# study-game-engines/directx-renderer-kurth

Hardware: AMD Instinct MI355X
Metric: physics steps/sec at 100k rigid bodies (higher is better)
Workload: dtype f32; 1 GPU; c3: 100k mixed colliders (sphere/capsule/OBB), dt 1/120 s, 30 solver iterations; bodies=100000, broadphase_pairs=611032, manifolds=251275, contacts=317267, joints=0, recoveries=0, parallelism=1 gpu

## Files before the change

directx-renderer-kurth_amd/csrc/k_broad.hip:

```cpp
#include "world.h"
#include <rocprim/rocprim.hpp>

#define CELL_BIAS (1 << 20)
#define CELL_MASK ((1u << 21) - 1u)
#define EMPTY_CELL 0xFFFFFFFFu

MI_DEV u64 packCell(i32 ix, i32 iy, i32 iz) { return ((u64)(u32)(ix & CELL_MASK)) | ((u64)(u32)(iy & CELL_MASK) << 21) | ((u64)(u32)(iz & CELL_MASK) << 42); }
MI_DEV u32 hashCell(u64 k, u32 mask)
{
	k ^= k >> 30; k *= 0xbf58476d1ce4e5b9ull; k ^= k >> 27; k *= 0x94d049bb133111ebull; k ^= k >> 31;
	return (u32)k & mask;
}
MI_DEV i32 cellCoord(float v, float invCell)
{
	float c = floorf(v * invCell);
	c = fminf(fmaxf(c, -(float)(CELL_BIAS - 2)), (float)(CELL_BIAS - 2));
	return (i32)c + CELL_BIAS;
}
MI_DEV u32 cellTag(i32 ix, i32 iy, i32 iz) { return ((u32)ix & 0x3FFu) | (((u32)iy & 0x3FFu) << 10) | (((u32)iz & 0x3FFu) << 20); }
MI_DEV bool aabbOverlap(float4 amin, float4 amax, float4 bmin, float4 bmax)
{
	if (amax.x < bmin.x || amin.x > bmax.x) return false;
	if (amax.y < bmin.y || amin.y > bmax.y) return false;
	if (amax.z < bmin.z || amin.z > bmax.z) return false;
	return true;
}

__global__ void __launch_bounds__(256) k_cell_assign(const u32* __restrict__ activeCols, u32 hashMask, const float4* __restrict__ aabbMin, const float4* __restrict__ aabbMax,
	u32* __restrict__ counters, u32* __restrict__ hashKey, u32* __restrict__ cellCount)
{
	const u32 gid = blockIdx.x * blockDim.x + threadIdx.x;
	if (gid == 0) { counters[CTR_FIRST_LARGE] = 0xFFFFFFFFu; counters[CTR_FIRST_INACTIVE] = 0xFFFFFFFFu; counters[CTR_PAIR_OVERFLOW] = 0u; }
	const u32 n = counters[CTR_ACTIVE_COLS];
	float maxExtent = fmaxf(__uint_as_float(counters[CTR_CELL_SIZE]), 1e-3f);
	float cell = maxExtent * 1.001f;
	float invCell = 1.f / cell;
	for (u32 a = gid; a < n; a += gridDim.x * blockDim.x)
	{
		const u32 i = activeCols[a];
		float4 mn = aabbMin[i], mx = aabbMax[i];
		float e = fmaxf(fmaxf(mx.x - mn.x, mx.y - mn.y), mx.z - mn.z);
		u32 h;
		if (mn.x > mx.x) { h = hashMask + 2; }
		else if (e > maxExtent) { h = hashMask + 1; }
		else { h = hashCell(packCell(cellCoord(mn.x, invCell), cellCoord(mn.y, invCell), cellCoord(mn.z, invCell)), hashMask); }
		hashKey[i] = h;
		atomicAdd(&cellCount[h], 1u);
	}
}

__global__ void __launch_bounds__(256) k_cell_place(const u32* __restrict__ counters, const u32* __restrict__ activeCols, const u32* __restrict__ hashKey, u32* __restrict__ cellBase, u32* __restrict__ tmpIdx)
{
	const u32 n = counters[CTR_ACTIVE_COLS];
	for (u32 a = blockIdx.x * blockDim.x + threadIdx.x; a < n; a += gridDim.x * blockDim.x) { const u32 i = activeCols[a]; tmpIdx[atomicAdd(&cellBase[hashKey[i]], 1u)] = i; }
}
__global__ void __launch_bounds__(256) k_cell_rank(u32* __restrict__ counters, u32 hashMask, const u32* __restrict__ hashKey, const u32* __restrict__ cellBase, const u32* __restrict__ cellCount, const u32* __restrict__ tmpIdx,
	const float4* __restrict__ aabbMin, const float4* __restrict__ aabbMax, float4* __restrict__ sBox, u32* __restrict__ cellRange)
{
	const u32 n = counters[CTR_ACTIVE_COLS];
	const float cell = fmaxf(__uint_as_float(counters[CTR_CELL_SIZE]), 1e-3f) * 1.001f;
	const float invCell = 1.f / cell;
	if (blockIdx.x == 0 && threadIdx.x == 0) counters[CTR_CELL_SIZE_USED] = counters[CTR_CELL_SIZE];
	for (u32 t = blockIdx.x * blockDim.x + threadIdx.x; t < n; t += gridDim.x * blockDim.x)
	{
		const u32 i = tmpIdx[t], h = hashKey[i], end = cellBase[h], start = end - cellCount[h];
		u32 rank = t - start;
		if (h != hashMask + 2u) { rank = 0; for (u32 u = start; u < end; ++u) rank += tmpIdx[u] < i ? 1u : 0u; }
		const u32 pos = start + rank;
		float4 mn = aabbMin[i], mx = aabbMax[i];
		mx.w = __uint_as_float(cellTag(cellCoord(mn.x, invCell), cellCoord(mn.y, invCell), cellCoord(mn.z, invCell)));
		mn.w = __uint_as_float(i);
		sBox[2 * pos] = mn; sBox[2 * pos + 1] = mx;
		if (t == start)
		{
			if (h <= hashMask) { cellRange[2 * h] = start; cellRange[2 * h + 1] = end; }
			else counters[h == hashMask + 1 ? CTR_FIRST_LARGE : CTR_FIRST_INACTIVE] = start;
		}
	}
}

#define PAIR_SLAB 32
#define PAIR_LANES 16
enum { MODE_SLAB = 0, MODE_WRITE = 1 };
template <int MODE>
__global__ void __launch_bounds__(256) k_pairs(u32 nc, u32 hashMask, const float4* __restrict__ sBox, const uint2* __restrict__ cellRange, u32* __restrict__ counters,
	u32* __restrict__ pairCount, const u32* __restrict__ pairOffset, uint2* __restrict__ out, u32 pairCap)
{
	u32 gid = blockIdx.x * blockDim.x + threadIdx.x;
	u32 t = gid / PAIR_LANES, g = gid % PAIR_LANES;
	bool valid = t < nc;
	u32 nEnd = min(counters[CTR_FIRST_INACTIVE], min(nc, counters[CTR_ACTIVE_COLS]));
	u32 firstLarge = min(counters[CTR_FIRST_LARGE], nEnd);
	bool live = valid && t < nEnd;
	if (MODE == MODE_WRITE) live = live && pairCount[t] > PAIR_SLAB;
	float4 amin = make_float4(0.f, 0.f, 0.f, 0.f), amax = amin;
	u32 me = 0;
	u32 s = 0, e = 0; u32 ntag = 0; bool checkKey = false;
	if (live)
	{
		amin = sBox[2 * t]; amax = sBox[2 * t + 1];
		me = __float_as_uint(amin.w);
		if (t >= firstLarge) { if (g == 0) { s = firstLarge; e = t; } }
		else if (g == 14) { s = firstLarge; e = nEnd; }
		else if (g < 14)
		{
			const float invCell = 1.f / (fmaxf(__uint_as_float(counters[CTR_CELL_SIZE_USED]), 1e-3f) * 1.001f);
			i32 ix = cellCoord(amin.x, invCell), iy = cellCoord(amin.y, invCell), iz = cellCoord(amin.z, invCell);
			i32 o = 13 + (i32)g;
			i32 dz = o / 9 - 1, dy = (o / 3) % 3 - 1, dx = o % 3 - 1;
			ntag = cellTag(ix + dx, iy + dy, iz + dz);
			u32 h = hashCell(packCell(ix + dx, iy + dy, iz + dz), hashMask);
			uint2 range = cellRange[h];
			if (range.x != EMPTY_CELL)
			{
				s = range.x; e = range.y;
				if (g == 0) e = min(e, t);
				checkKey = true;
			}
		}
	}
	u32 n = 0;
	u32 hit0 = 0, hit1 = 0, hit2 = 0, hit3 = 0;
	for (u32 u = s; u < e; u += 4u)
	{
		float4 bmin[4], bmax[4];
#pragma unroll
		for (u32 k = 0; k < 4u; ++k) if (u + k < e) { bmin[k] = sBox[2 * (u + k)]; bmax[k] = sBox[2 * (u + k) + 1]; }
#pragma unroll
		for (u32 k = 0; k < 4u; ++k)
		{
			if (u + k >= e) continue;
			if (checkKey && __float_as_uint(bmax[k].w) != ntag) continue;
			if (aabbOverlap(amin, amax, bmin[k], bmax[k]))
			{
				u32 partner = __float_as_uint(bmin[k].w);
				if (n == 0) hit0 = partner; else if (n == 1) hit1 = partner; else if (n == 2) hit2 = partner; else if (n == 3) hit3 = partner;
				++n;
			}
		}
	}
	u32 incl = n;
	for (u32 d = 1; d < PAIR_LANES; d <<= 1) { u32 v = __shfl_up(incl, d, PAIR_LANES); if (g >= d) incl += v; }
	u32 total = __shfl(incl, PAIR_LANES - 1, PAIR_LANES);
	u32 pos = incl - n;
	if (MODE == MODE_SLAB && valid && g == 0) { pairCount[t] = live ? total : 0; if (total > PAIR_SLAB) counters[CTR_PAIR_OVERFLOW] = 1; }
	if (!n) return;
	size_t base = (MODE == MODE_WRITE) ? (size_t)pairOffset[t] : (size_t)t * PAIR_SLAB;
	u32 room = (MODE == MODE_WRITE) ? 0xFFFFFFFFu : PAIR_SLAB;
	if (n <= 4)
	{
		for (u32 k = 0; k < n; ++k)
		{
			u32 partner = k == 0 ? hit0 : (k == 1 ? hit1 : (k == 2 ? hit2 : hit3));
			if (pos + k < room && (MODE == MODE_SLAB || base + pos + k < pairCap)) out[base + pos + k] = make_uint2(me, partner);
		}
		return;
	}
	for (u32 u = s; u < e; ++u)
	{
		float4 bmin = sBox[2 * u], bmax = sBox[2 * u + 1];
		if (checkKey && __float_as_uint(bmax.w) != ntag) continue;
		if (!aabbOverlap(amin, amax, bmin, bmax)) continue;
		if (pos < room && (MODE == MODE_SLAB || base + pos < pairCap)) out[base + pos] = make_uint2(me, __float_as_uint(bmin.w));
		++pos;
	}
}

__global__ void __launch_bounds__(256) k_pairs_pack(u32 nc, const u32* __restrict__ pairCount, const u32* __restrict__ pairOffset, const uint2* __restrict__ slab,
	uint2* __restrict__ pairs, u32 pairCap)
{
	u32 i = blockIdx.x * blockDim.x + threadIdx.x;
	u32 t = i / PAIR_SLAB, k = i % PAIR_SLAB;
	if (t >= nc || k >= pairCount[t]) return;
	u32 dst = pairOffset[t] + k;
	if (dst < pairCap) pairs[dst] = slab[i];
}

__global__ void k_finish_pair_count(u32 launched, const u32* __restrict__ pairCount, const u32* __restrict__ pairOffset, u32* __restrict__ counters, const double* __restrict__ sapPartial, u32 sapBlocks, u32 stepParity)
{
	double acc[7] = { 0., 0., 0., 0., 0., 0., 0. };
	for (u32 b = threadIdx.x; b < sapBlocks; b += 64u) for (int k = 0; k < 7; ++k) acc[k] += sapPartial[(size_t)b * 7 + k];
	for (int o = 32; o > 0; o >>= 1) for (int k = 0; k < 7; ++k) acc[k] += __shfl_xor(acc[k], o);
	if (threadIdx.x == 0 && blockIdx.x == 0)
	{
		const u32 na = counters[CTR_ACTIVE_COLS], nc = min(na, launched);
		counters[CTR_ACTIVE_OVERFLOW] = na > launched ? 1u : 0u;
		counters[CTR_NUM_PAIRS] = nc ? pairOffset[nc - 1] + pairCount[nc - 1] : 0;
		counters[CTR_CELL_SIZE] = 0;
		const double n = acc[6] > 0. ? acc[6] : 1.;
		const double vx = acc[3] - acc[0] * acc[0] / n, vy = acc[4] - acc[1] * acc[1] / n, vz = acc[5] - acc[2] * acc[2] / n;
		counters[CTR_SAP_AXIS + (stepParity ^ 1u)] = (vx > vy) ? ((vx > vz) ? 0u : 2u) : ((vy > vz) ? 1u : 2u);
	}
}

static void ensureTemp(World& w, size_t bytes)
{
	if (bytes > w.tempStorage.cap) w.tempStorage.ensure(bytes + bytes / 2 + 4096, w.stream);
}
void prim_sort_pairs_u32(World& w, const u32* kin, u32* kout, const u32* vin, u32* vout, u32 n, u32 bits)
{
	if (!n) return;
	size_t bytes = 0;
	MI_CHECK(rocprim::radix_sort_pairs(nullptr, bytes, kin, kout, vin, vout, n, 0, bits, w.stream));
	ensureTemp(w, bytes);
	MI_CHECK(rocprim::radix_sort_pairs(w.tempStorage.p, bytes, kin, kout, vin, vout, n, 0, bits, w.stream));
}
void prim_sort_pairs_u32_u64(World& w, const u32* kin, u32* kout, const u64* vin, u64* vout, u32 n, u32 bits)
{
	if (!n) return;
	size_t bytes = 0;
	MI_CHECK(rocprim::radix_sort_pairs(nullptr, bytes, kin, kout, vin, vout, n, 0, bits, w.stream));
	ensureTemp(w, bytes);
	MI_CHECK(rocprim::radix_sort_pairs(w.tempStorage.p, bytes, kin, kout, vin, vout, n, 0, bits, w.stream));
}
void prim_exclusive_scan_u32(World& w, const u32* in, u32* out, u32 n)
{
	if (!n) return;
	size_t bytes = 0;
	MI_CHECK(rocprim::exclusive_scan(nullptr, bytes, in, out, 0u, n, rocprim::plus<u32>(), w.stream));
	ensureTemp(w, bytes);
	MI_CHECK(rocprim::exclusive_scan(w.tempStorage.p, bytes, in, out, 0u, n, rocprim::plus<u32>(), w.stream));
}

static u32 log2ceil(u32 v) { u32 b = 0; while ((1u << b) < v) ++b; return b; }

void launch_broadphase_count(World& w)
{
	if (!w.nc) return;
	const u32 bound = (u32)std::min<u64>(w.nc, (u64)w.estActiveCols + w.estActiveCols / 8u + 2048u);
	w.pairBound = bound;
	dim3 grid(std::max(1u, (bound + 255u) / 256u)), block(256);
	u32 H = w.hashTableSize, mask = H - 1;
	hipLaunchKernelGGL(k_cell_assign, grid, block, 0, w.stream, w.actCols.p, mask, w.aabbMin.p, w.aabbMax.p, w.dCounters.p, w.hashKey.p, w.cellCount.p);
	prim_exclusive_scan_u32(w, w.cellCount.p, w.cellBase.p, H + 3);
	hipLaunchKernelGGL(k_cell_place, grid, block, 0, w.stream, w.dCounters.p, w.actCols.p, w.hashKey.p, w.cellBase.p, w.sortIdx.p);
	hipLaunchKernelGGL(k_cell_rank, grid, block, 0, w.stream, w.dCounters.p, mask, w.hashKey.p, w.cellBase.p, w.cellCount.p, w.sortIdx.p, w.aabbMin.p, w.aabbMax.p, w.sBox.p, w.cellStart.p);
	w.pairSlab.ensure((size_t)bound * PAIR_SLAB, w.stream);
	if (w.lastError) return;
	hipLaunchKernelGGL(HIP_KERNEL_NAME(k_pairs<MODE_SLAB>), dim3((u32)(((size_t)bound * PAIR_LANES + 255) / 256)), block, 0, w.stream, bound, mask, w.sBox.p, (const uint2*)w.cellStart.p, w.dCounters.p,
		w.pairCount.p, w.pairOffset.p, w.pairSlab.p, 0u);
	prim_exclusive_scan_u32(w, w.pairCount.p, w.pairOffset.p, bound);
	hipLaunchKernelGGL(k_finish_pair_count, dim3(1), dim3(64), 0, w.stream, bound, w.pairCount.p, w.pairOffset.p, w.dCounters.p, w.sapPartial.p, w.sapBlocks, w.stats.numInternalSteps & 1u);
}

void launch_broadphase_write(World& w, u32 numPairs, bool slabOverflow)
{
	const u32 nc = w.pairBound;
	if (!nc || !numPairs) return;
	hipLaunchKernelGGL(k_pairs_pack, dim3((u32)(((size_t)nc * PAIR_SLAB + 255) / 256)), dim3(256), 0, w.stream, nc, w.pairCount.p, w.pairOffset.p, w.pairSlab.p, w.pairs.p, (u32)w.pairCap);
	if (slabOverflow)
		hipLaunchKernelGGL(HIP_KERNEL_NAME(k_pairs<MODE_WRITE>), dim3((u32)(((size_t)nc * PAIR_LANES + 255) / 256)), dim3(256), 0, w.stream, nc, w.hashTableSize - 1, w.sBox.p, (const uint2*)w.cellStart.p, w.dCounters.p, w.pairCount.p, w.pairOffset.p, w.pairs.p, (u32)w.pairCap);
}
```

Before: 528.2 steps/s.

## Balance broadphase pair scan across lanes and skip unreachable neighbor cells

```diff
diff --git a/directx-renderer-kurth_amd/csrc/k_broad.hip b/directx-renderer-kurth_amd/csrc/k_broad.hip
--- a/directx-renderer-kurth_amd/csrc/k_broad.hip
+++ b/directx-renderer-kurth_amd/csrc/k_broad.hip
@@ -81,13 +81,18 @@
 
 #define PAIR_SLAB 32
 #define PAIR_LANES 16
+#define PAIR_NO_TAG 0xFFFFFFFFu
 enum { MODE_SLAB = 0, MODE_WRITE = 1 };
+MI_DEV uint2 pairRange(const uint4* ranges, u32 r) { return make_uint2(ranges[r].x, ranges[r].y); }
+MI_DEV const float4* pairBox(const float4* __restrict__ sBox, u32 u) { return (const float4*)((const char*)sBox + u * 32u); }
 template <int MODE>
 __global__ void __launch_bounds__(256) k_pairs(u32 nc, u32 hashMask, const float4* __restrict__ sBox, const uint2* __restrict__ cellRange, u32* __restrict__ counters,
 	u32* __restrict__ pairCount, const u32* __restrict__ pairOffset, uint2* __restrict__ out, u32 pairCap)
 {
+	__shared__ uint4 sRange[256 / PAIR_LANES][PAIR_LANES];
 	u32 gid = blockIdx.x * blockDim.x + threadIdx.x;
 	u32 t = gid / PAIR_LANES, g = gid % PAIR_LANES;
+	const uint4* __restrict__ ranges = sRange[threadIdx.x / PAIR_LANES];
 	bool valid = t < nc;
 	u32 nEnd = min(counters[CTR_FIRST_INACTIVE], min(nc, counters[CTR_ACTIVE_COLS]));
 	u32 firstLarge = min(counters[CTR_FIRST_LARGE], nEnd);
@@ -95,47 +100,69 @@
 	if (MODE == MODE_WRITE) live = live && pairCount[t] > PAIR_SLAB;
 	float4 amin = make_float4(0.f, 0.f, 0.f, 0.f), amax = amin;
 	u32 me = 0;
-	u32 s = 0, e = 0; u32 ntag = 0; bool checkKey = false;
+	u32 s = 0, len = 0, ntag = PAIR_NO_TAG;
 	if (live)
 	{
 		amin = sBox[2 * t]; amax = sBox[2 * t + 1];
 		me = __float_as_uint(amin.w);
-		if (t >= firstLarge) { if (g == 0) { s = firstLarge; e = t; } }
-		else if (g == 14) { s = firstLarge; e = nEnd; }
+		if (t >= firstLarge) { if (g == 0) { s = firstLarge; len = t - firstLarge; } }
+		else if (g == 14) { s = firstLarge; len = nEnd - firstLarge; }
 		else if (g < 14)
 		{
 			const float invCell = 1.f / (fmaxf(__uint_as_float(counters[CTR_CELL_SIZE_USED]), 1e-3f) * 1.001f);
 			i32 ix = cellCoord(amin.x, invCell), iy = cellCoord(amin.y, invCell), iz = cellCoord(amin.z, invCell);
 			i32 o = 13 + (i32)g;
 			i32 dz = o / 9 - 1, dy = (o / 3) % 3 - 1, dx = o % 3 - 1;
-			ntag = cellTag(ix + dx, iy + dy, iz + dz);
-			u32 h = hashCell(packCell(ix + dx, iy + dy, iz + dz), hashMask);
-			uint2 range = cellRange[h];
-			if (range.x != EMPTY_CELL)
+			bool reach = true;
+			if (dx > 0 && cellCoord(amax.x, invCell) == ix) reach = false;
+			if (dy > 0 && cellCoord(amax.y, invCell) == iy) reach = false;
+			if (dz > 0 && cellCoord(amax.z, invCell) == iz) reach = false;
+			if (reach)
 			{
-				s = range.x; e = range.y;
-				if (g == 0) e = min(e, t);
-				checkKey = true;
+				ntag = cellTag(ix + dx, iy + dy, iz + dz);
+				u32 h = hashCell(packCell(ix + dx, iy + dy, iz + dz), hashMask);
+				uint2 range = cellRange[h];
+				if (range.x != EMPTY_CELL) { s = range.x; const u32 e = g == 0 ? min(range.y, t) : range.y; len = e > s ? e - s : 0u; }
 			}
 		}
 	}
+	u32 end = len;
+	for (u32 d = 1; d < PAIR_LANES; d <<= 1) { u32 v = __shfl_up(end, d, PAIR_LANES); if (g >= d) end += v; }
+	sRange[threadIdx.x / PAIR_LANES][g] = make_uint4(end, s - (end - len), ntag, 0u);
+	__syncthreads();
+	const u32 T = ranges[PAIR_LANES - 1].x;
+	const u32 chunk = (T + PAIR_LANES - 1u) / PAIR_LANES;
+	const u32 lo = min(g * chunk, T), hi = min(lo + chunk, T);
+	u32 r0 = 0;
+#pragma unroll
+	for (u32 k = 0; k < PAIR_LANES - 1u; ++k) r0 += ranges[k].x <= lo ? 1u : 0u;
 	u32 n = 0;
 	u32 hit0 = 0, hit1 = 0, hit2 = 0, hit3 = 0;
-	for (u32 u = s; u < e; u += 4u)
-	{
-		float4 bmin[4], bmax[4];
+	if (lo < hi)
+	{
+		u32 r = r0; uint2 cur = pairRange(ranges, r);
+		for (u32 p = lo; p < hi; p += 4u)
+		{
+			float4 bmin[4], bmax[4]; u32 from = 0;
 #pragma unroll
-		for (u32 k = 0; k < 4u; ++k) if (u + k < e) { bmin[k] = sBox[2 * (u + k)]; bmax[k] = sBox[2 * (u + k) + 1]; }
+			for (u32 k = 0; k < 4u; ++k) if (p + k < hi)
+			{
+				while (p + k >= cur.x) cur = pairRange(ranges, ++r);
+				const float4* box = pairBox(sBox, cur.y + p + k);
+				from |= r << (4u * k); bmin[k] = box[0]; bmax[k] = box[1];
+			}
 #pragma unroll
-		for (u32 k = 0; k < 4u; ++k)
-		{
-			if (u + k >= e) continue;
-			if (checkKey && __float_as_uint(bmax[k].w) != ntag) continue;
-			if (aabbOverlap(amin, amax, bmin[k], bmax[k]))
+			for (u32 k = 0; k < 4u; ++k)
 			{
-				u32 partner = __float_as_uint(bmin[k].w);
-				if (n == 0) hit0 = partner; else if (n == 1) hit1 = partner; else if (n == 2) hit2 = partner; else if (n == 3) hit3 = partner;
-				++n;
+				if (p + k >= hi) continue;
+				const u32 want = ranges[(from >> (4u * k)) & 15u].z;
+				if (want != PAIR_NO_TAG && __float_as_uint(bmax[k].w) != want) continue;
+				if (aabbOverlap(amin, amax, bmin[k], bmax[k]))
+				{
+					u32 partner = __float_as_uint(bmin[k].w);
+					if (n == 0) hit0 = partner; else if (n == 1) hit1 = partner; else if (n == 2) hit2 = partner; else if (n == 3) hit3 = partner;
+					++n;
+				}
 			}
 		}
 	}
@@ -156,10 +183,14 @@
 		}
 		return;
 	}
-	for (u32 u = s; u < e; ++u)
-	{
-		float4 bmin = sBox[2 * u], bmax = sBox[2 * u + 1];
-		if (checkKey && __float_as_uint(bmax.w) != ntag) continue;
+	u32 r = r0; uint2 cur = pairRange(ranges, r);
+	for (u32 p = lo; p < hi; ++p)
+	{
+		while (p >= cur.x) cur = pairRange(ranges, ++r);
+		const float4* box = pairBox(sBox, cur.y + p);
+		float4 bmin = box[0], bmax = box[1];
+		const u32 want = ranges[r].z;
+		if (want != PAIR_NO_TAG && __float_as_uint(bmax.w) != want) continue;
 		if (!aabbOverlap(amin, amax, bmin, bmax)) continue;
 		if (pos < room && (MODE == MODE_SLAB || base + pos < pairCap)) out[base + pos] = make_uint2(me, __float_as_uint(bmin.w));
 		++pos;
```

New measurement: 543.3 steps/s (median of 6 runs). 2.9% higher.
